# FJingxian/JanusX

Hardware: AMD Instinct MI355X
Metric: SNPs/sec full -lmm (GRM+eig+scan) (higher is better)
Workload: dtype f64 (eigendecomposition, REML and per-SNP statistics; GRM and rotation products are exact int8 / split-f16 MFMA sums merged in f64)

## Files before the change

janusx_amd/csrc/k_rotate_i8.hip:

```cpp
#include <stdlib.h>

#include "jx_common.h"

namespace jx {

typedef int i32x4 __attribute__((ext_vector_type(4)));
typedef int i32x16 __attribute__((ext_vector_type(16)));
typedef uint32_t u32x4q __attribute__((ext_vector_type(4)));

constexpr int RI_TM = 256;
constexpr int RI_TN = 128;
constexpr int RI_BK = 64;
constexpr int RI_IMG_A = RI_TM * RI_BK;
constexpr int RI_IMG_B = RI_TN * RI_BK;
constexpr int RI_SET = RI_IMG_A + 3 * RI_IMG_B;

__device__ __forceinline__ int ri_chunk_off(int row, int chunk) { return row * 64 + ((chunk ^ ((row >> 2) & 3)) << 4); }

__device__ __forceinline__ u32x4q ri_decode16(uint32_t w) {
    const uint32_t hi = (w >> 1) & 0x55555555u;
    const uint32_t v = hi + (hi & w);
    u32x4q o;
    o.x = v & 0x03030303u;
    o.y = (v >> 2) & 0x03030303u;
    o.z = (v >> 4) & 0x03030303u;
    o.w = (v >> 6) & 0x03030303u;
    return o;
}

__device__ __forceinline__ u32x4q ri_decode16_missing(uint32_t w) {
    const uint32_t v = w & ~(w >> 1) & 0x55555555u;
    u32x4q o;
    o.x = v & 0x03030303u;
    o.y = (v >> 2) & 0x03030303u;
    o.z = (v >> 4) & 0x03030303u;
    o.w = (v >> 6) & 0x03030303u;
    return o;
}

__global__ __launch_bounds__(256) void ut_rowmax_kernel(const float *__restrict__ ut, int n, int npad, float *__restrict__ umax) {
    const int j = blockIdx.x * 4 + (threadIdx.x >> 6), lane = threadIdx.x & 63;
    if (j >= npad) return;
    float a = 0.0f;
    if (j < n)
        for (int i = lane; i < n; i += 64) a = fmaxf(a, fabsf(ut[(int64_t)j * n + i]));
#pragma unroll
    for (int off = 32; off > 0; off >>= 1) a = fmaxf(a, __shfl_xor(a, off, 64));
    if (lane == 0) umax[j] = (a > 0.0f && a < 3.0e38f) ? a : 1.0f;
}

__global__ __launch_bounds__(256) void ut_quant3_kernel(const float *__restrict__ ut, int n, int64_t npad,
                                                        const float *__restrict__ umax, int8_t *__restrict__ q) {
    const int64_t idx = (int64_t)blockIdx.x * blockDim.x + threadIdx.x;
    const int64_t groups = npad / 16;
    if (idx >= npad * groups) return;
    const int64_t j = idx / groups, gq = idx - j * groups;
    int8_t o[3][16];
    const double inv = (j < n) ? 1.0 / (double)umax[j] : 0.0;
#pragma unroll
    for (int pos = 0; pos < 16; ++pos) {
        const int smp = ((pos & 3) << 2) | (pos >> 2);
        const int64_t i = gq * 16 + smp;
        double u = 0.0;
        if (j < n && i < n) u = (double)ut[j * (int64_t)n + i] * inv;
        const double a1 = u * 127.0;
        double q1 = rint(a1);
        const double a2 = (a1 - q1) * 254.0;
        double q2 = rint(a2);
        const double a3 = (a2 - q2) * 254.0;
        double q3 = rint(a3);
        q1 = fmin(fmax(q1, -127.0), 127.0);
        q2 = fmin(fmax(q2, -127.0), 127.0);
        q3 = fmin(fmax(q3, -127.0), 127.0);
        o[0][pos] = (int8_t)q1;
        o[1][pos] = (int8_t)q2;
        o[2][pos] = (int8_t)q3;
    }
#pragma unroll
    for (int pl = 0; pl < 3; ++pl)
        *reinterpret_cast<uint4 *>(q + pl * npad * npad + j * npad + gq * 16) = *reinterpret_cast<const uint4 *>(o[pl]);
}

template <int MODE>
__global__ __launch_bounds__(512, 2) void rotate_i8_kernel(const uint8_t *__restrict__ p32, int64_t m_total,
                                                           const int32_t *__restrict__ rows, int nrows,
                                                           const uint4 *__restrict__ lut16, const float *__restrict__ rowoff,
                                                           const float *__restrict__ usum, const int8_t *__restrict__ q,
                                                           const float *__restrict__ umax, int64_t npad, int n,
                                                           float *__restrict__ out, int64_t ldo,
                                                           const int32_t *__restrict__ sel) {
    extern __shared__ __attribute__((aligned(16))) uint8_t ri_smem[];
    float *sOff = reinterpret_cast<float *>(ri_smem + 2 * RI_SET);
    float *sSgn = sOff + RI_TM;
    int *sPos = reinterpret_cast<int *>(sSgn + RI_TM);

    const int tid = threadIdx.x, lane = tid & 63, wave = tid >> 6;
    const int wm = wave >> 2, wn = wave & 3;
    const int nrt = (nrows + RI_TM - 1) / RI_TM;
    const int xcd = blockIdx.x & 7, local = blockIdx.x >> 3;
    const int ct = (local / nrt) * 8 + xcd;
    if ((int64_t)ct * RI_TN >= npad) return;
    const int j0 = ct * RI_TN;
    const int r0 = (local % nrt) * RI_TM;

    const int arow = tid >> 1, ahalf = tid & 1;
    const uint8_t *arec = p32;
    int row_exact = 1;
    {
        const int r = r0 + arow;
        float boff = 0.0f, sgn = 1.0f;
        int pos = -1;
        if (r < nrows) {
            pos = sel ? sel[r] : r;
            const int64_t rec = rows ? (int64_t)rows[pos] : (int64_t)pos;
            arec = p32 + rec * 32;
            const float t = rowoff[pos];
            if (MODE == 1) {
                boff = t;
            } else {
                row_exact = (t == t) ? 1 : 0;
                const bool flipped = (lut16[pos].x & 0xffffu) != 0u;
                sgn = flipped ? -1.0f : 1.0f;
                boff = row_exact ? (t + (flipped ? 2.0f : 0.0f)) : 0.0f;
            }
        }
        if (ahalf == 0) {
            sOff[arow] = boff;
            sSgn[arow] = sgn;
            sPos[arow] = pos;
        }
    }
    if (__syncthreads_and(row_exact) == 0) return;
    arec += 8 * ahalf;

    const int brow = tid >> 2, bpart = tid & 3;
    const bool bok = j0 + brow < npad;
    const int8_t *bsrc = q + (int64_t)(bok ? j0 + brow : 0) * npad + bpart * 16;
    const uint32_t bmask = bok ? 0xffffffffu : 0u;
    const int64_t plane = npad * npad;
    const int boff_lds = ri_chunk_off(brow, bpart);

    uint2 wa = make_uint2(0, 0);
    u32x4q b0, b1, b2;
    auto load_a = [&](int kstep) {
        const int tile = kstep >> 1, sub = kstep & 1;
        wa = *reinterpret_cast<const uint2 *>(arec + (int64_t)tile * m_total * 32 + sub * 16);
    };
    auto load_b = [&](int64_t kcol) {
        b0 = *reinterpret_cast<const u32x4q *>(bsrc + kcol);
        b1 = *reinterpret_cast<const u32x4q *>(bsrc + plane + kcol);
        b2 = *reinterpret_cast<const u32x4q *>(bsrc + 2 * plane + kcol);
    };
    auto stage = [&](uint8_t *set) {
        *reinterpret_cast<u32x4q *>(set + ri_chunk_off(arow, 2 * ahalf)) = MODE == 1 ? ri_decode16_missing(wa.x) : ri_decode16(wa.x);
        *reinterpret_cast<u32x4q *>(set + ri_chunk_off(arow, 2 * ahalf + 1)) = MODE == 1 ? ri_decode16_missing(wa.y) : ri_decode16(wa.y);
        const u32x4q mk = {bmask, bmask, bmask, bmask};
        *reinterpret_cast<u32x4q *>(set + RI_IMG_A + boff_lds) = b0 & mk;
        *reinterpret_cast<u32x4q *>(set + RI_IMG_A + RI_IMG_B + boff_lds) = b1 & mk;
        *reinterpret_cast<u32x4q *>(set + RI_IMG_A + 2 * RI_IMG_B + boff_lds) = b2 & mk;
    };

    i32x16 acc[3][4];
#pragma unroll
    for (int pl = 0; pl < 3; ++pl)
#pragma unroll
        for (int mi = 0; mi < 4; ++mi)
#pragma unroll
            for (int r = 0; r < 16; ++r) acc[pl][mi][r] = 0;

    const int h = lane >> 5, frow = lane & 31;
    auto mfma_ks = [&](const uint8_t *set, int ks) {
        i32x4 b[3];
#pragma unroll
        for (int pl = 0; pl < 3; ++pl)
            b[pl] = *reinterpret_cast<const i32x4 *>(set + RI_IMG_A + pl * RI_IMG_B + ri_chunk_off(wn * 32 + frow, 2 * ks + h));
#pragma unroll
        for (int mp = 0; mp < 2; ++mp) {
            i32x4 a[2];
#pragma unroll
            for (int u = 0; u < 2; ++u)
                a[u] = *reinterpret_cast<const i32x4 *>(set + ri_chunk_off(wm * 128 + (2 * mp + u) * 32 + frow, 2 * ks + h));
#pragma unroll
            for (int u = 0; u < 2; ++u)
#pragma unroll
                for (int pl = 0; pl < 3; ++pl)
                    acc[pl][2 * mp + u] = __builtin_amdgcn_mfma_i32_32x32x32_i8(a[u], b[pl], acc[pl][2 * mp + u], 0, 0, 0);
            if (mp == 0) __builtin_amdgcn_sched_barrier(0);
        }
    };

    const int nk = (int)(npad / RI_BK);
    load_a(0);
    load_b(0);
    stage(ri_smem);
    {
        const int k1 = nk > 1 ? 1 : 0;
        load_a(k1);
        load_b((int64_t)k1 * RI_BK);
    }
    __syncthreads();
    int cur = 0;
    for (int ks = 0; ks < nk; ++ks) {
        const uint8_t *rd = ri_smem + cur * RI_SET;
        uint8_t *wr = ri_smem + (cur ^ 1) * RI_SET;
        const int kn = ks + 2 < nk ? ks + 2 : nk - 1;
        mfma_ks(rd, 0);
        stage(wr);
        load_a(kn);
        load_b((int64_t)kn * RI_BK);
        __builtin_amdgcn_sched_barrier(0);
        mfma_ks(rd, 1);
        __syncthreads();
        cur ^= 1;
    }

    const int gj = j0 + wn * 32 + frow;
    const bool colok = gj < n;
    const double um = colok ? (double)umax[gj] : 0.0;
    const double w1 = um / 127.0, w2 = um / (127.0 * 254.0), w3 = um / (127.0 * 254.0 * 254.0);
    const float us = (MODE == 0 && colok) ? usum[gj] : 0.0f;
#pragma unroll
    for (int mi = 0; mi < 4; ++mi) {
#pragma unroll
        for (int r = 0; r < 16; ++r) {
            const int lr = wm * 128 + mi * 32 + (r & 3) + 8 * (r >> 2) + 4 * h;
            const int gr = sPos[lr];
            if (gr >= 0 && colok) {
                const double v = (double)acc[0][mi][r] * w1 + (double)acc[1][mi][r] * w2 + (double)acc[2][mi][r] * w3;
                float *dst = out + (int64_t)gr * ldo + gj;
                if (MODE == 1) *dst = fmaf(sOff[lr], (float)v, *dst);
                else *dst = fmaf(sOff[lr], us, sSgn[lr] * (float)v);
            }
        }
    }
}

constexpr int RD_BK = 128;
constexpr int RD_A = 8 * 1024;
constexpr int RD_B = RI_TN * RD_BK;
constexpr int RD_STAGE = RD_A + 3 * RD_B;

__device__ __forceinline__ void rd_glds(const void *base, uint32_t off, unsigned lds_dst) {
    unsigned keep;
    const uint64_t b = (uint64_t)(uintptr_t)base;
    const uint32_t blo = __builtin_amdgcn_readfirstlane((uint32_t)b), bhi = __builtin_amdgcn_readfirstlane((uint32_t)(b >> 32));
    const uint64_t sb = ((uint64_t)bhi << 32) | blo;
    asm volatile("s_mov_b32 %0, m0\n\ts_mov_b32 m0, %3\n\ts_nop 0\n\tglobal_load_lds_dwordx4 %1, %2\n\ts_mov_b32 m0, %0"
                 : "=&s"(keep)
                 : "v"(off), "s"(sb), "s"(__builtin_amdgcn_readfirstlane(lds_dst))
                 : "memory");
}

template <int MODE> __device__ __forceinline__ i32x4 rd_decode(uint32_t w) {
    const u32x4q o = MODE == 1 ? ri_decode16_missing(w) : ri_decode16(w);
    i32x4 r;
    r.x = (int)o.x;
    r.y = (int)o.y;
    r.z = (int)o.z;
    r.w = (int)o.w;
    return r;
}

template <int MODE>
__global__ __launch_bounds__(512, 2) void rotate_i8_dma_kernel(const uint8_t *__restrict__ p32, int64_t m_total,
                                                               const int32_t *__restrict__ rows, int nrows,
                                                               const uint4 *__restrict__ lut16, const float *__restrict__ rowoff,
                                                               const float *__restrict__ usum, const int8_t *__restrict__ q,
                                                               const float *__restrict__ umax, int64_t npad, int n,
                                                               float *__restrict__ out, int64_t ldo,
                                                               const int32_t *__restrict__ sel) {
    extern __shared__ __attribute__((aligned(16))) uint8_t rd_smem[];
    float *sOff = reinterpret_cast<float *>(rd_smem + 2 * RD_STAGE);
    float *sSgn = sOff + RI_TM;
    int *sPos = reinterpret_cast<int *>(sSgn + RI_TM);

    const int tid = threadIdx.x, lane = tid & 63, wave = tid >> 6;
    const int wm = wave >> 2, wn = wave & 3;
    const int nrt = (nrows + RI_TM - 1) / RI_TM;
    const int xcd = blockIdx.x & 7, local = blockIdx.x >> 3;
    const int ct = (local / nrt) * 8 + xcd;
    if ((int64_t)ct * RI_TN >= npad) return;
    const int j0 = ct * RI_TN;
    const int r0 = (local % nrt) * RI_TM;

    uint32_t aoff = 0;
    int row_exact = 1;
    {
        const int arow = 32 * wave + (lane & 31);
        const int r = r0 + arow;
        float boff = 0.0f, sgn = 1.0f;
        int pos = -1;
        if (r < nrows) {
            pos = sel ? sel[r] : r;
            aoff = (uint32_t)(rows ? rows[pos] : pos) * 32u;
            const float t = rowoff[pos];
            if (MODE == 1) {
                boff = t;
            } else {
                row_exact = (t == t) ? 1 : 0;
                const bool flipped = (lut16[pos].x & 0xffffu) != 0u;
                sgn = flipped ? -1.0f : 1.0f;
                boff = row_exact ? (t + (flipped ? 2.0f : 0.0f)) : 0.0f;
            }
        }
        if (lane < 32) {
            sOff[arow] = boff;
            sSgn[arow] = sgn;
            sPos[arow] = pos;
        }
    }
    if (__syncthreads_and(row_exact) == 0) return;
    aoff += 16u * (uint32_t)(lane >> 5);

    uint32_t boffs[2];
#pragma unroll
    for (int e = 0; e < 2; ++e) {
        const int col = 16 * wave + 8 * e + (lane >> 3);
        const int c = (lane & 7) ^ ((col >> 1) & 7);
        boffs[e] = (uint32_t)col * (uint32_t)npad + (uint32_t)c * 16u;
    }
    const int8_t *qtile = q + (int64_t)j0 * npad;
    const int64_t plane = npad * npad;
    const int64_t atile = m_total * 32;
    const unsigned lds0 = (unsigned)(uintptr_t)rd_smem;
    auto issue = [&](int t, int buf) {
        const unsigned st = lds0 + buf * RD_STAGE;
        rd_glds(p32 + (int64_t)t * atile, aoff, st + wave * 1024);
#pragma unroll
        for (int pl = 0; pl < 3; ++pl)
#pragma unroll
            for (int e = 0; e < 2; ++e)
                rd_glds(qtile + pl * plane + (int64_t)t * RD_BK, boffs[e], st + RD_A + pl * RD_B + (2 * wave + e) * 1024);
    };

    i32x16 acc[3][4];
#pragma unroll
    for (int pl = 0; pl < 3; ++pl)
#pragma unroll
        for (int mi = 0; mi < 4; ++mi)
#pragma unroll
            for (int r = 0; r < 16; ++r) acc[pl][mi][r] = 0;

    const int h = lane >> 5, frow = lane & 31;
    const int afrag = wm * 4 * 1024 + h * 512 + frow * 16;
    const int bcol = (wn * 32 + frow) * RD_BK;
    const int bx0 = (4 * h) ^ ((frow >> 1) & 7);

    const int nk = (int)(npad / RD_BK);
    issue(0, 0);
    int buf = 0;
    for (int t = 0; t < nk; ++t) {
        asm volatile("s_waitcnt vmcnt(0)" ::: "memory");
        __builtin_amdgcn_s_barrier();
        asm volatile("" ::: "memory");
        issue(t + 1 < nk ? t + 1 : nk - 1, buf ^ 1);
        const uint8_t *st = rd_smem + buf * RD_STAGE;
        i32x4 araw[4];
#pragma unroll
        for (int mi = 0; mi < 4; ++mi) araw[mi] = *reinterpret_cast<const i32x4 *>(st + afrag + mi * 1024);
#pragma unroll
        for (int ks = 0; ks < 4; ++ks) {
            i32x4 b[3];
#pragma unroll
            for (int pl = 0; pl < 3; ++pl)
                b[pl] = *reinterpret_cast<const i32x4 *>(st + RD_A + pl * RD_B + bcol + ((bx0 ^ ks) << 4));
#pragma unroll
            for (int mi = 0; mi < 4; ++mi) {
                const i32x4 a = rd_decode<MODE>((uint32_t)araw[mi][ks]);
#pragma unroll
                for (int pl = 0; pl < 3; ++pl)
                    acc[pl][mi] = __builtin_amdgcn_mfma_i32_32x32x32_i8(a, b[pl], acc[pl][mi], 0, 0, 0);
            }
        }
        buf ^= 1;
    }
    asm volatile("s_waitcnt vmcnt(0)" ::: "memory");

    const int gj = j0 + wn * 32 + frow;
    const bool colok = gj < n;
    const double um = colok ? (double)umax[gj] : 0.0;
    const double w1 = um / 127.0, w2 = um / (127.0 * 254.0), w3 = um / (127.0 * 254.0 * 254.0);
    const float us = (MODE == 0 && colok) ? usum[gj] : 0.0f;
#pragma unroll
    for (int mi = 0; mi < 4; ++mi) {
#pragma unroll
        for (int r = 0; r < 16; ++r) {
            const int lr = wm * 128 + mi * 32 + (r & 3) + 8 * (r >> 2) + 4 * h;
            const int gr = sPos[lr];
            if (gr >= 0 && colok) {
                const double v = (double)acc[0][mi][r] * w1 + (double)acc[1][mi][r] * w2 + (double)acc[2][mi][r] * w3;
                float *dst = out + (int64_t)gr * ldo + gj;
                if (MODE == 1) *dst = fmaf(sOff[lr], (float)v, *dst);
                else *dst = fmaf(sOff[lr], us, sSgn[lr] * (float)v);
            }
        }
    }
}

static bool rot_i8_dma() {
    static const bool on = !(getenv("JXGPU_ROT_I8_DMA") && atoi(getenv("JXGPU_ROT_I8_DMA")) == 0);
    return on;
}

extern float g_last_ms[24];

}

using namespace jx;

namespace jx {
int launch_rotate_i8_missing(hipStream_t st, const uint8_t *d_p32, int64_t m_total, int n, const int32_t *d_rows, const int32_t *d_sel,
                             int nsel, const float *d_rowmiss, const int8_t *d_q, const float *d_umax, float *d_out, int64_t ld_out);
}
extern "C" int jxg_rotate_missing_dense(const uint8_t *d_p32, int64_t m_total, int n, const int32_t *d_rows, const int32_t *d_sel,
                                        int nsel, const float *d_rowmiss, const int8_t *d_q, const float *d_umax, float *d_out,
                                        int64_t ld_out, void *stream) {
    return launch_rotate_i8_missing((hipStream_t)stream, d_p32, m_total, n, d_rows, d_sel, nsel, d_rowmiss, d_q, d_umax, d_out, ld_out);
}

extern "C" int jxg_ut_quant3(const float *d_ut, int n, int8_t *d_q, float *d_umax, void *stream) {
    hipStream_t st = (hipStream_t)stream;
    const int64_t npad = (int64_t)num_tiles(n) * JXG_TILE;
    hipLaunchKernelGGL(ut_rowmax_kernel, dim3((unsigned)((npad + 3) / 4)), dim3(256), 0, st, d_ut, n, (int)npad, d_umax);
    JX_LAUNCH_CHECK();
    const int64_t items = npad * (npad / 16);
    if ((items + 255) / 256 > 0x7fffffffLL) return fail("jxg_ut_quant3: grid too large");
    hipLaunchKernelGGL(ut_quant3_kernel, dim3((unsigned)((items + 255) / 256)), dim3(256), 0, st, d_ut, n, npad, d_umax, d_q);
    JX_LAUNCH_CHECK();
    return 0;
}

namespace jx {
int launch_rotate_i8(hipStream_t st, const uint8_t *d_p32, int64_t m_total, int n, const int32_t *d_rows, const int32_t *d_sel,
                     int nsel, const void *d_lut16, const float *d_rowoff, const float *d_usum, const int8_t *d_q,
                     const float *d_umax, float *d_out, int64_t ld_out) {
    if (nsel <= 0) return 0;
    const int nt = num_tiles(n);
    const int64_t npad = (int64_t)nt * JXG_TILE;
    if (!d_q || !d_umax || !d_rowoff || !d_usum || n > 66000) return fail("launch_rotate_i8: planes missing or n > 66000");
    const int nrows = nsel;
    const int nct = (int)((npad + RI_TN - 1) / RI_TN), nrt = (nrows + RI_TM - 1) / RI_TM;
    static bool attr = false;
    const int lds = 2 * RI_SET + 3072;
    if (!attr) {
        JX_HIP(hipFuncSetAttribute((const void *)rotate_i8_kernel<0>, hipFuncAttributeMaxDynamicSharedMemorySize, lds));
        JX_HIP(hipFuncSetAttribute((const void *)rotate_i8_kernel<1>, hipFuncAttributeMaxDynamicSharedMemorySize, lds));
        attr = true;
    }
    dim3 grid((unsigned)(((nct + 7) / 8) * 8 * nrt));
    if (rot_i8_dma() && m_total < (1LL << 27)) {
        static bool attr_dma = false;
        const int lds_dma = 2 * RD_STAGE + 3072;
        if (!attr_dma) {
            JX_HIP(hipFuncSetAttribute((const void *)rotate_i8_dma_kernel<0>, hipFuncAttributeMaxDynamicSharedMemorySize, lds_dma));
            attr_dma = true;
        }
        hipLaunchKernelGGL(rotate_i8_dma_kernel<0>, grid, dim3(512), lds_dma, st, d_p32, m_total, d_rows, nrows,
                           (const uint4 *)d_lut16, d_rowoff, d_usum, d_q, d_umax, npad, n, d_out, ld_out, d_sel);
        JX_LAUNCH_CHECK();
        return 0;
    }
    hipLaunchKernelGGL(rotate_i8_kernel<0>, grid, dim3(512), lds, st, d_p32, m_total, d_rows, nrows, (const uint4 *)d_lut16,
                       d_rowoff, d_usum, d_q, d_umax, npad, n, d_out, ld_out, d_sel);
    JX_LAUNCH_CHECK();
    return 0;
}

int launch_rotate_i8_missing(hipStream_t st, const uint8_t *d_p32, int64_t m_total, int n, const int32_t *d_rows, const int32_t *d_sel,
                             int nsel, const float *d_rowmiss, const int8_t *d_q, const float *d_umax, float *d_out, int64_t ld_out) {
    if (nsel <= 0) return 0;
    const int nt = num_tiles(n);
    const int64_t npad = (int64_t)nt * JXG_TILE;
    if (!d_q || !d_umax || !d_rowmiss || !d_sel || n > 66000) return fail("launch_rotate_i8_missing: planes / list missing or n > 66000");
    const int nct = (int)((npad + RI_TN - 1) / RI_TN), nrt = (nsel + RI_TM - 1) / RI_TM;
    static bool attr = false;
    const int lds = 2 * RI_SET + 3072;
    if (!attr) {
        JX_HIP(hipFuncSetAttribute((const void *)rotate_i8_kernel<1>, hipFuncAttributeMaxDynamicSharedMemorySize, lds));
        attr = true;
    }
    dim3 grid((unsigned)(((nct + 7) / 8) * 8 * nrt));
    if (rot_i8_dma() && m_total < (1LL << 27)) {
        static bool attr_dma = false;
        const int lds_dma = 2 * RD_STAGE + 3072;
        if (!attr_dma) {
            JX_HIP(hipFuncSetAttribute((const void *)rotate_i8_dma_kernel<1>, hipFuncAttributeMaxDynamicSharedMemorySize, lds_dma));
            attr_dma = true;
        }
        hipLaunchKernelGGL(rotate_i8_dma_kernel<1>, grid, dim3(512), lds_dma, st, d_p32, m_total, d_rows, nsel,
                           (const uint4 *)nullptr, d_rowmiss, (const float *)nullptr, d_q, d_umax, npad, n, d_out, ld_out, d_sel);
        JX_LAUNCH_CHECK();
        return 0;
    }
    hipLaunchKernelGGL(rotate_i8_kernel<1>, grid, dim3(512), lds, st, d_p32, m_total, d_rows, nsel, (const uint4 *)nullptr,
                       d_rowmiss, (const float *)nullptr, d_q, d_umax, npad, n, d_out, ld_out, d_sel);
    JX_LAUNCH_CHECK();
    return 0;
}
}
```

janusx_amd/switches.py:

```python

SWITCHES = {
    "JXGPU_OZ_PLANES": ("numerics", "6 (5 inside pipeline.eigh_from_grm(f32_consumer=True))",
                        "digit planes of the sliced int8 products of the eigensolver (4..6); 4 is NOT a product state",
                        "test_sliced_int8_gemm[5|6], test_full_size_c2/c3/c4_properties[f32_consumer], test_end_to_end_two_stage"),
    "JXGPU_EIGH_F32_PLANES": ("numerics", "5", "0 keeps 6 planes for the f32-consuming pipeline",
                              "test_full_size_c3_properties[0.0-False] (6) / [0.0-True] (5)"),
    "JXGPU_STEDC_OZ_PLANES": ("numerics", "unset (follows JXGPU_OZ_PLANES)", "planes of the divide-and-conquer merges alone", "untested"),
    "JXGPU_GRM_MISS_DIGITS": ("numerics", "3", "2 = the two-digit dense missing-call GRM of rounds 4-5 (beta off by 1e-5..1e-4 end to end)",
                              "test_end_to_end_two_stage (default); 2 is NOT a product state"),
    "JXGPU_GRM_MISS": ("numerics", "1", "0: rows with missing calls on the fp16 split kernel (f32 accumulation, like the reference)",
                       "test_grm_missing_calls_sparse_correction"),
    "JXGPU_GRM_MISS_MAX": ("numerics", "0.012", "largest missing share for the sparse correction", "test_grm_missing_calls_sparse_correction"),
    "JXGPU_GRM_MISS_DENSE_MIN": ("numerics", "0.0015", "missing share from which the dense digit form replaces the sparse correction",
                                 "test_grm_missing_calls_sparse_correction, scripts/diag_e2e_two_stage.py"),
    "JXGPU_GRM_MISS_DENSE_ROWS": ("numerics", "16384", "fewest SNPs for the dense digit form", "test_grm_missing_calls_sparse_correction"),
    "JXGPU_GRM_FP4": ("form", "0", "1: the count Gram of the 256-tile form on the fp4 matrix pipes from a nibble image (exact like the int8 kernel)",
                      "test_grm_count_gram_on_the_fp4_pipes"),
    "JXGPU_GRM_I8": ("numerics", "1", "0: exact-integer SNPs on the fp16 single-product kernel (f32 sums instead of exact i32)", "untested"),
    "JXGPU_GRM_EXACT": ("numerics", "1", "0: every SNP on the fp16 hi/lo split kernel", "untested"),
    "JXGPU_ROT_I8": ("numerics", "1", "0: design rows on the fp16 hi/lo rotation instead of the exact int8 planes",
                     "test_full_size_rotation_kernels_with_mixed_rows"),
    "JXGPU_ROT_EXACT": ("numerics", "1", "0: no integer-LUT fast path in the fp16 rotation", "untested"),
    "JXGPU_ROT_MISS_DENSE": ("numerics", "auto", "form of the missing-call term of the int8 rotation (both exact)",
                             "test_rotation_rows_with_a_few_missing_calls_take_the_exact_path"),
    "JXGPU_ROT_MISS_MAX": ("numerics", "auto", "missing calls per row up to which the gather form is taken",
                           "test_rotation_rows_with_a_few_missing_calls_take_the_exact_path"),
    "JXGPU_PCG_I8": ("numerics", "1", "0: the PCG / HE operator halves on the f32 bit-plane table kernels (f32 partial sums per tile) instead of "
                     "exact int8 plane sums of a four-digit image of the vector", "test_pcg_operator_forms_agree"),
    "JXGPU_FVLMM_FUSED": ("numerics", "1", "0 / 2: unfused / always-fused fixed-lambda scan (f64 sums in a different order + f32 G~ round trip)",
                          "test_fixed_lambda_scan_fused_into_the_rotation_epilogue"),
    "JXGPU_SCAN_EXACT": ("numerics", "unset", "reference-formulation scan kernel instead of the tabulated one (1e-9 apart)",
                         "test_fast_scan_matches_exact_scan (through the entry points)"),
    "JXGPU_SCAN_SERIES": ("numerics", "1", "0: no per-SNP Chebyshev series (3e-16 apart)", "test_fast_scan_matches_exact_scan"),
    "JXGPU_SCAN_INTERP": ("numerics", "1", "0: Brent evaluates the tabulated objective directly instead of its per-SNP Chebyshev interpolant "
                          "(3.7e-15 apart; dim <= 4, series form only)",
                          "test_warm_start_chain_device_pipeline_matches_trajectories, test_fast_scan_matches_exact_scan, full-size legs"),
    "JXGPU_LMM2_EXACT": ("numerics", "unset", "LMM2 on the reference-formulation kernel", "test_lmm2_routes"),
    "JXGPU_EIGH": ("numerics", "auto", "onestage | twostage | rocsolver: which eigensolver (eigenvectors differ within 1e-10)",
                   "test_eigh_two_stage_path_and_its_fallback"),
    "JXGPU_EIGH_TWOSTAGE_MIN": ("numerics", "1500", "size from which the two-stage reduction runs", "test_eigh_two_stage_path_and_its_fallback"),
    "JXGPU_STEDC": ("numerics", "own", "rocsolver: vendor divide and conquer (diagnostic)", "test_eigh_own_divide_and_conquer"),
    "JXGPU_ORMTR": ("numerics", "own", "rocsolver back-transformation (diagnostic)", "untested"),
    "JXGPU_ORMTR_OZ": ("numerics", "1", "0: Q1 on the f64 MFMA GEMM instead of the sliced int8 one", "untested"),
    "JXGPU_STEDC_OZ": ("numerics", "1", "0: merges on the f64 MFMA GEMM", "untested"),
    "JXGPU_OZ_MIN_N": ("numerics", "3000 / 750", "size from which Q1 / the merges take the sliced products", "untested"),
    "JXGPU_DIST_BACKEND": ("knob", "nccl", "collective backend of `jx` multi-rank runs", "test_cli_two_ranks_share_one_gpu"),
    "JXGPU_DIST_EIGH": ("knob", "1", "0: replicated eigendecomposition on several ranks", "test_bench_two_ranks_share_one_gpu"),
    "JXGPU_DIST_EIGH_MIN_N": ("knob", "16384", "size from which the eigensolver's stages are dealt over the ranks", "test_bench_two_ranks_share_one_gpu"),
    "JXGPU_DIST_EIGH_ONESTAGE": ("knob", "unset", "sharded one-stage reduction", "untested"),
    "JXGPU_DIST_BAND": ("knob", "1", "0: band reduction replicated", "untested"),
    "JXGPU_DIST_BAND_MIN_N": ("knob", "16384", "size from which the band reduction is sharded", "test_sharded_band_reduction_rccl_single_rank"),
    "JXGPU_DIST_BAND_BLOCK": ("test", "auto", "block rows of the sharded band reduction", "test_sharded_band_reduction_rccl_single_rank"),
    "JXGPU_DIST_DC_WINDOW": ("knob", "1", "0: top-level merge replicated", "untested"),
    "JXGPU_SYR2K_PIPE_WGS": ("knob", "7/8 of the CUs", "workgroups of the persistent rank-2k update (the rest of the CUs serve the panel chain)",
                             "test_rank_2k_update_forms_give_the_same_bits"),
    "JXGPU_SPLMM_ROUTE": ("knob", "auto", "dense | block | factor: form of K + lambda I of the sparse-GRM routes",
                          "test_splmm_block_route_matches_the_dense_route, test_splmm_giant_component_both_sides_of_the_limit"),
    "JXGPU_SPLMM_BLOCK": ("knob", "4096", "samples per diagonal block of the block route", "test_splmm_block_route_matches_the_dense_route"),
    "JXGPU_SPLMM_BLOCK_MIN_N": ("knob", "16384", "size from which the block route is taken", "untested"),
    "JXGPU_SPGRM_ACC_GB": ("knob", "auto", "HBM for the sparse-GRM builder's accumulator", "untested"),
    "JXGPU_SPECTRAL_CACHE": ("knob", "1", "0: no reuse of the last sparse GRM's decomposition", "untested"),
    **{k: ("form", "default", "kernel / launch shape of the same computation", t) for k, t in {
        "JXGPU_BC_OWNED": "test_bulge_chasing_position_owned_equals_sweep_owned", "JXGPU_SB2ST_WGS": "untested", "JXGPU_GRM_I8_TILE": "test_sparse_grm_row_panels_write_the_same_file",
        "JXGPU_GRM_TILE": "untested", "JXGPU_GRM_EXACT_BK": "untested", "JXGPU_ROT256": "untested", "JXGPU_SCAN_NOLDS": "untested",
        "JXGPU_SCAN_NOTILE": "untested", "JXGPU_SBBACK_BAL": "untested", "JXGPU_SBBACK_BAL5": "test_eigh_balanced_q2_forms",
        "JXGPU_SBBACK_BAL_MIN": "untested", "JXGPU_SBBACK_BAL_PER": "untested", "JXGPU_SBBACK_GROUPS": "untested", "JXGPU_SBBACK_NW": "untested",
        "JXGPU_SBBACK_PAIR": "untested", "JXGPU_SBBACK_SOLO": "untested", "JXGPU_STEDC_LEAF": "test_eigh_own_divide_and_conquer",
        "JXGPU_STEDC_OWNLEAF": "untested", "JXGPU_STEDC_PAR": "untested", "JXGPU_STEDC_PARMIN": "untested", "JXGPU_SY2SB_LOOKAHEAD": "untested",
        "JXGPU_SYTRD_KT": "untested", "JXGPU_SYTRD_SYR2K": "untested", "JXGPU_SYTRD_TAIL": "untested", "JXGPU_SYTRD_TARGET": "untested",
        "JXGPU_DSYMM_SLOTS": "untested", "JXGPU_DSYMM_SPLIT": "untested", "JXGPU_ORMTR_NB": "untested",
        "JXGPU_ROT_I8_DMA": "test_int8_rotation_forms_give_the_same_bits",
        "JXGPU_SCAN_CHAIN_SPLIT": "test_warm_start_chain_kernels_on_rotated_rows_with_invalid_rows",
        "JXGPU_REPACK_WINDOW": "test_repack_of_a_sample_subset_window_form",
        "JXGPU_SYR2K_PIPE": "test_rank_2k_update_forms_give_the_same_bits",
        "JXGPU_KING_TILE": "test_fused_path_finds_every_finite_pair"}.items()},
    "JXGPU_QB_SKIP": ("test", "unset", "skips parts of the Q2 kernel (timing ablation; results are WRONG)", "test_q2_staggered_units_equal_lockstep (the lockstep value 64 only)"),
    "JXGPU_BC_SKIP": ("test", "unset", "bulge-chasing ablation (results WRONG)", "untested"),
    "JXGPU_BO_SLEEP": ("test", "unset", "hand-off delay of the bulge chasing (timing)", "untested"),
    "JXGPU_EIGH_TRACE": ("trace", "unset", "stage times of a decomposition to stderr", "-"),
    "JXGPU_PCG_TRACE": ("trace", "unset", "set-up marks of the PCG / HE / staging paths", "-"),
    "JXGPU_BENCH_BACKEND": ("test", "nccl", "bench.py: gloo for ranks sharing a GPU", "test_bench_two_ranks_share_one_gpu"),
    "JXGPU_BENCH_STEP_SLEEP_MS": ("test", "unset", "bench.py diagnostic: idle time in front of every odd step", "-"),
    "JXGPU_BENCH_CHILD": ("test", "unset", "bench.py: marks a child process", "-"),
    "JXGPU_BENCH_FORCE_DIST": ("test", "unset", "bench.py: one rank on the multi-rank code path", "test_distributed_eigh_rccl_callback_single_rank"),
    "JXGPU_DIST_EIGH_FORCE": ("test", "unset", "sharded eigensolver forms with one rank", "test_sharded_band_reduction_rccl_single_rank"),
    "JXGPU_DIST_EIGH_TEST_DISAGREE": ("test", "unset", "fault injection of the replica agreement check", "test_distributed_eigh_two_ranks_share_one_gpu"),
    "JXGPU_DIST_EIGH_TEST_DISAGREE2": ("test", "unset", "fault injection of the replica agreement check", "test_distributed_eigh_two_ranks_share_one_gpu"),
    "JXGPU_PCG_TEST_FAIL": ("test", "unset", "fault injection of the marker-sharded PCG", "test_marker_sharded_pcg_two_ranks_share_one_gpu"),
    "JXGPU_SCAN_CHAIN_FORCE_DIRECT": ("test", "unset", "row of a chain scan forced onto direct evaluations (its chain takes the one-kernel form)",
                                      "test_warm_start_chain_kernels_on_rotated_rows_with_invalid_rows"),
    "JXGPU_SPLMM_COMPONENT_MAX": ("test", "auto", "component limit of the spectral sparse routes", "test_splmm_giant_component_both_sides_of_the_limit"),
    "JXGPU_SPGRM_PANEL_ROWS": ("test", "auto", "row panels of the sparse-GRM builder", "test_sparse_grm_row_panels_write_the_same_file"),
}


def markdown_table(classes=("numerics",)):
    rows = ["| switch | product value | what another value does | covered by |", "|---|---|---|---|"]
    for name, (cls, default, what, test) in sorted(SWITCHES.items()):
        if cls in classes:
            cell = lambda t: str(t).replace(" | ", " / ").replace("|", "/")
            rows.append(f"| `{name}` | {cell(default)} | {cell(what)} | {cell(test)} |")
    return "\n".join(rows)
```

Baseline: 141,800.

## Add 512x64 rotation tile with grouped block order and interleaved DMA issue

The int8 rotation DMA kernel is templated on tile shape and gains a 512x64 tile, picked automatically when there are enough tiles to fill the device's CUs. Block-to-tile mapping for the narrow tile groups row and column tiles per XCD to improve L2 reuse. Next-stage global-to-LDS loads are now spread between the MFMA groups, with scheduling barriers, instead of issued all at once. The changed tile shape shifts the A/B reuse ratio and LDS size, which may affect occupancy, and blocks whose columns lie past n now exit early.

After: 143,200, median of 6. Within noise of the previous version (+1.0%).

```diff
diff --git a/janusx_amd/csrc/k_rotate_i8.hip b/janusx_amd/csrc/k_rotate_i8.hip
--- a/janusx_amd/csrc/k_rotate_i8.hip
+++ b/janusx_amd/csrc/k_rotate_i8.hip
@@ -1,4 +1,5 @@
 #include <stdlib.h>
+#include <string.h>
 
 #include "jx_common.h"
 
@@ -236,9 +237,17 @@
 }
 
 constexpr int RD_BK = 128;
-constexpr int RD_A = 8 * 1024;
-constexpr int RD_B = RI_TN * RD_BK;
-constexpr int RD_STAGE = RD_A + 3 * RD_B;
+
+template <int TM, int TN> struct RdTile {
+    static constexpr int WM = TM / 128, WN = TN / 32;
+    static constexpr int A = TM * 32;
+    static constexpr int B = TN * RD_BK;
+    static constexpr int STAGE = A + 3 * B;
+    static constexpr int NA = TM / 256;
+    static constexpr int NB = TN / 64;
+    static constexpr int LDS = 2 * STAGE + 3 * TM * 4;
+    static_assert(WM * WN == 8 && NA >= 1 && NB >= 1, "8 waves of 128 x 32");
+};
 
 __device__ __forceinline__ void rd_glds(const void *base, uint32_t off, unsigned lds_dst) {
     unsigned keep;
@@ -261,7 +270,7 @@
     return r;
 }
 
-template <int MODE>
+template <int MODE, int TM, int TN>
 __global__ __launch_bounds__(512, 2) void rotate_i8_dma_kernel(const uint8_t *__restrict__ p32, int64_t m_total,
                                                                const int32_t *__restrict__ rows, int nrows,
                                                                const uint4 *__restrict__ lut16, const float *__restrict__ rowoff,
@@ -269,38 +278,53 @@
                                                                const float *__restrict__ umax, int64_t npad, int n,
                                                                float *__restrict__ out, int64_t ldo,
                                                                const int32_t *__restrict__ sel) {
+    using T = RdTile<TM, TN>;
     extern __shared__ __attribute__((aligned(16))) uint8_t rd_smem[];
-    float *sOff = reinterpret_cast<float *>(rd_smem + 2 * RD_STAGE);
-    float *sSgn = sOff + RI_TM;
-    int *sPos = reinterpret_cast<int *>(sSgn + RI_TM);
+    float *sOff = reinterpret_cast<float *>(rd_smem + 2 * T::STAGE);
+    float *sSgn = sOff + TM;
+    int *sPos = reinterpret_cast<int *>(sSgn + TM);
 
     const int tid = threadIdx.x, lane = tid & 63, wave = tid >> 6;
-    const int wm = wave >> 2, wn = wave & 3;
-    const int nrt = (nrows + RI_TM - 1) / RI_TM;
+    const int wm = wave / T::WN, wn = wave % T::WN;
+    const int nrt = (nrows + TM - 1) / TM;
     const int xcd = blockIdx.x & 7, local = blockIdx.x >> 3;
-    const int ct = (local / nrt) * 8 + xcd;
-    if ((int64_t)ct * RI_TN >= npad) return;
-    const int j0 = ct * RI_TN;
-    const int r0 = (local % nrt) * RI_TM;
-
-    uint32_t aoff = 0;
+    int rt, ct;
+    if (TN == 64) {
+        const int srt = (nrt + 7) >> 3;
+        const int s = (local >> 5) * 8 + xcd, w = local & 31;
+        rt = (s % srt) * 8 + (w & 7);
+        ct = (s / srt) * 4 + (w >> 3);
+        if (rt >= nrt) return;
+    } else {
+        rt = local % nrt;
+        ct = (local / nrt) * 8 + xcd;
+    }
+    if ((int64_t)ct * TN >= npad) return;
+    const int j0 = ct * TN;
+    if (j0 >= n) return;
+    const int r0 = rt * TM;
+
+    uint32_t aoff[T::NA];
     int row_exact = 1;
-    {
-        const int arow = 32 * wave + (lane & 31);
+#pragma unroll
+    for (int e = 0; e < T::NA; ++e) {
+        const int arow = 32 * (wave + 8 * e) + (lane & 31);
         const int r = r0 + arow;
         float boff = 0.0f, sgn = 1.0f;
         int pos = -1;
+        aoff[e] = 0;
         if (r < nrows) {
             pos = sel ? sel[r] : r;
-            aoff = (uint32_t)(rows ? rows[pos] : pos) * 32u;
+            aoff[e] = (uint32_t)(rows ? rows[pos] : pos) * 32u;
             const float t = rowoff[pos];
             if (MODE == 1) {
                 boff = t;
             } else {
-                row_exact = (t == t) ? 1 : 0;
+                const int exact = (t == t) ? 1 : 0;
+                row_exact &= exact;
                 const bool flipped = (lut16[pos].x & 0xffffu) != 0u;
                 sgn = flipped ? -1.0f : 1.0f;
-                boff = row_exact ? (t + (flipped ? 2.0f : 0.0f)) : 0.0f;
+                boff = exact ? (t + (flipped ? 2.0f : 0.0f)) : 0.0f;
             }
         }
         if (lane < 32) {
@@ -308,14 +332,14 @@
             sSgn[arow] = sgn;
             sPos[arow] = pos;
         }
+        aoff[e] += 16u * (uint32_t)(lane >> 5);
     }
     if (__syncthreads_and(row_exact) == 0) return;
-    aoff += 16u * (uint32_t)(lane >> 5);
-
-    uint32_t boffs[2];
-#pragma unroll
-    for (int e = 0; e < 2; ++e) {
-        const int col = 16 * wave + 8 * e + (lane >> 3);
+
+    uint32_t boffs[T::NB];
+#pragma unroll
+    for (int e = 0; e < T::NB; ++e) {
+        const int col = 8 * (T::NB * wave + e) + (lane >> 3);
         const int c = (lane & 7) ^ ((col >> 1) & 7);
         boffs[e] = (uint32_t)col * (uint32_t)npad + (uint32_t)c * 16u;
     }
@@ -323,14 +347,15 @@
     const int64_t plane = npad * npad;
     const int64_t atile = m_total * 32;
     const unsigned lds0 = (unsigned)(uintptr_t)rd_smem;
-    auto issue = [&](int t, int buf) {
-        const unsigned st = lds0 + buf * RD_STAGE;
-        rd_glds(p32 + (int64_t)t * atile, aoff, st + wave * 1024);
-#pragma unroll
-        for (int pl = 0; pl < 3; ++pl)
-#pragma unroll
-            for (int e = 0; e < 2; ++e)
-                rd_glds(qtile + pl * plane + (int64_t)t * RD_BK, boffs[e], st + RD_A + pl * RD_B + (2 * wave + e) * 1024);
+    constexpr int NP = T::NA + 3 * T::NB;
+    auto issue_piece = [&](int t, int buf, int i) {
+        const unsigned st = lds0 + buf * T::STAGE;
+        if (i < T::NA) {
+            rd_glds(p32 + (int64_t)t * atile, aoff[i], st + (wave + 8 * i) * 1024);
+        } else {
+            const int pl = (i - T::NA) / T::NB, e = (i - T::NA) % T::NB;
+            rd_glds(qtile + pl * plane + (int64_t)t * RD_BK, boffs[e], st + T::A + pl * T::B + (T::NB * wave + e) * 1024);
+        }
     };
 
     i32x16 acc[3][4];
@@ -347,14 +372,15 @@
     const int bx0 = (4 * h) ^ ((frow >> 1) & 7);
 
     const int nk = (int)(npad / RD_BK);
-    issue(0, 0);
+#pragma unroll
+    for (int i = 0; i < NP; ++i) issue_piece(0, 0, i);
     int buf = 0;
     for (int t = 0; t < nk; ++t) {
         asm volatile("s_waitcnt vmcnt(0)" ::: "memory");
         __builtin_amdgcn_s_barrier();
         asm volatile("" ::: "memory");
-        issue(t + 1 < nk ? t + 1 : nk - 1, buf ^ 1);
-        const uint8_t *st = rd_smem + buf * RD_STAGE;
+        const int tn = t + 1 < nk ? t + 1 : nk - 1;
+        const uint8_t *st = rd_smem + buf * T::STAGE;
         i32x4 araw[4];
 #pragma unroll
         for (int mi = 0; mi < 4; ++mi) araw[mi] = *reinterpret_cast<const i32x4 *>(st + afrag + mi * 1024);
@@ -363,13 +389,18 @@
             i32x4 b[3];
 #pragma unroll
             for (int pl = 0; pl < 3; ++pl)
-                b[pl] = *reinterpret_cast<const i32x4 *>(st + RD_A + pl * RD_B + bcol + ((bx0 ^ ks) << 4));
+                b[pl] = *reinterpret_cast<const i32x4 *>(st + T::A + pl * T::B + bcol + ((bx0 ^ ks) << 4));
 #pragma unroll
             for (int mi = 0; mi < 4; ++mi) {
                 const i32x4 a = rd_decode<MODE>((uint32_t)araw[mi][ks]);
 #pragma unroll
                 for (int pl = 0; pl < 3; ++pl)
                     acc[pl][mi] = __builtin_amdgcn_mfma_i32_32x32x32_i8(a, b[pl], acc[pl][mi], 0, 0, 0);
+                if (ks * 4 + mi < NP) {
+                    __builtin_amdgcn_sched_barrier(0);
+                    issue_piece(tn, buf ^ 1, ks * 4 + mi);
+                    __builtin_amdgcn_sched_barrier(0);
+                }
             }
         }
         buf ^= 1;
@@ -400,6 +431,63 @@
 static bool rot_i8_dma() {
     static const bool on = !(getenv("JXGPU_ROT_I8_DMA") && atoi(getenv("JXGPU_ROT_I8_DMA")) == 0);
     return on;
+}
+
+constexpr int RD_WIDE_MIN_ROUNDS = 1;
+
+static int rot_i8_tile_switch() {
+    const char *e = getenv("JXGPU_ROT_I8_TILE");
+    if (!e || !*e) return 0;
+    if (!strcmp(e, "256x128")) return 1;
+    if (!strcmp(e, "512x64")) return 2;
+    return -1;
+}
+
+static int device_cus() {
+    static int cus = 0;
+    if (!cus) {
+        int dev = 0;
+        hipDeviceProp_t prop;
+        if (hipGetDevice(&dev) != hipSuccess || hipGetDeviceProperties(&prop, dev) != hipSuccess) return 256;
+        cus = prop.multiProcessorCount > 0 ? prop.multiProcessorCount : 256;
+    }
+    return cus;
+}
+
+static bool rot_i8_tile_512(int nrows, int n) {
+    return (int64_t)((nrows + 511) / 512) * ((n + 63) / 64) >= (int64_t)RD_WIDE_MIN_ROUNDS * device_cus();
+}
+
+template <int MODE, int TM, int TN>
+static int launch_rd(hipStream_t st, const uint8_t *d_p32, int64_t m_total, const int32_t *d_rows, int nrows, const uint4 *d_lut16,
+                     const float *d_rowoff, const float *d_usum, const int8_t *d_q, const float *d_umax, int64_t npad, int n,
+                     float *d_out, int64_t ld_out, const int32_t *d_sel) {
+    using T = RdTile<TM, TN>;
+    static bool attr = false;
+    if (!attr) {
+        JX_HIP(hipFuncSetAttribute((const void *)rotate_i8_dma_kernel<MODE, TM, TN>, hipFuncAttributeMaxDynamicSharedMemorySize, T::LDS));
+        attr = true;
+    }
+    const int64_t nct = (npad + TN - 1) / TN, nrt = (nrows + TM - 1) / TM;
+    const int64_t wgs = TN == 64 ? ((((nrt + 7) / 8) * ((nct + 3) / 4) + 7) / 8) * 8 * 32 : ((nct + 7) / 8) * 8 * nrt;
+    if (wgs > 0x7fffffffLL) return fail("rotate_i8: grid too large");
+    hipLaunchKernelGGL((rotate_i8_dma_kernel<MODE, TM, TN>), dim3((unsigned)wgs), dim3(512), T::LDS, st, d_p32, m_total, d_rows, nrows,
+                       d_lut16, d_rowoff, d_usum, d_q, d_umax, npad, n, d_out, ld_out, d_sel);
+    JX_LAUNCH_CHECK();
+    return 0;
+}
+
+template <int MODE>
+static int launch_rd_tile(hipStream_t st, const uint8_t *d_p32, int64_t m_total, const int32_t *d_rows, int nrows, const uint4 *d_lut16,
+                          const float *d_rowoff, const float *d_usum, const int8_t *d_q, const float *d_umax, int64_t npad, int n,
+                          float *d_out, int64_t ld_out, const int32_t *d_sel) {
+    const int sw = rot_i8_tile_switch();
+    if (sw < 0) return fail("JXGPU_ROT_I8_TILE: 256x128 or 512x64");
+    if (sw ? sw == 2 : rot_i8_tile_512(nrows, n))
+        return launch_rd<MODE, 512, 64>(st, d_p32, m_total, d_rows, nrows, d_lut16, d_rowoff, d_usum, d_q, d_umax, npad, n, d_out, ld_out,
+                                        d_sel);
+    return launch_rd<MODE, 256, 128>(st, d_p32, m_total, d_rows, nrows, d_lut16, d_rowoff, d_usum, d_q, d_umax, npad, n, d_out, ld_out,
+                                     d_sel);
 }
 
 extern float g_last_ms[24];
@@ -448,18 +536,9 @@
         attr = true;
     }
     dim3 grid((unsigned)(((nct + 7) / 8) * 8 * nrt));
-    if (rot_i8_dma() && m_total < (1LL << 27)) {
-        static bool attr_dma = false;
-        const int lds_dma = 2 * RD_STAGE + 3072;
-        if (!attr_dma) {
-            JX_HIP(hipFuncSetAttribute((const void *)rotate_i8_dma_kernel<0>, hipFuncAttributeMaxDynamicSharedMemorySize, lds_dma));
-            attr_dma = true;
-        }
-        hipLaunchKernelGGL(rotate_i8_dma_kernel<0>, grid, dim3(512), lds_dma, st, d_p32, m_total, d_rows, nrows,
-                           (const uint4 *)d_lut16, d_rowoff, d_usum, d_q, d_umax, npad, n, d_out, ld_out, d_sel);
-        JX_LAUNCH_CHECK();
-        return 0;
-    }
+    if (rot_i8_dma() && m_total < (1LL << 27))
+        return launch_rd_tile<0>(st, d_p32, m_total, d_rows, nrows, (const uint4 *)d_lut16, d_rowoff, d_usum, d_q, d_umax, npad, n, d_out,
+                                 ld_out, d_sel);
     hipLaunchKernelGGL(rotate_i8_kernel<0>, grid, dim3(512), lds, st, d_p32, m_total, d_rows, nrows, (const uint4 *)d_lut16,
                        d_rowoff, d_usum, d_q, d_umax, npad, n, d_out, ld_out, d_sel);
     JX_LAUNCH_CHECK();
@@ -480,18 +559,9 @@
         attr = true;
     }
     dim3 grid((unsigned)(((nct + 7) / 8) * 8 * nrt));
-    if (rot_i8_dma() && m_total < (1LL << 27)) {
-        static bool attr_dma = false;
-        const int lds_dma = 2 * RD_STAGE + 3072;
-        if (!attr_dma) {
-            JX_HIP(hipFuncSetAttribute((const void *)rotate_i8_dma_kernel<1>, hipFuncAttributeMaxDynamicSharedMemorySize, lds_dma));
-            attr_dma = true;
-        }
-        hipLaunchKernelGGL(rotate_i8_dma_kernel<1>, grid, dim3(512), lds_dma, st, d_p32, m_total, d_rows, nsel,
-                           (const uint4 *)nullptr, d_rowmiss, (const float *)nullptr, d_q, d_umax, npad, n, d_out, ld_out, d_sel);
-        JX_LAUNCH_CHECK();
-        return 0;
-    }
+    if (rot_i8_dma() && m_total < (1LL << 27))
+        return launch_rd_tile<1>(st, d_p32, m_total, d_rows, nsel, (const uint4 *)nullptr, d_rowmiss, (const float *)nullptr, d_q, d_umax,
+                                 npad, n, d_out, ld_out, d_sel);
     hipLaunchKernelGGL(rotate_i8_kernel<1>, grid, dim3(512), lds, st, d_p32, m_total, d_rows, nsel, (const uint4 *)nullptr,
                        d_rowmiss, (const float *)nullptr, d_q, d_umax, npad, n, d_out, ld_out, d_sel);
     JX_LAUNCH_CHECK();
diff --git a/janusx_amd/switches.py b/janusx_amd/switches.py
--- a/janusx_amd/switches.py
+++ b/janusx_amd/switches.py
@@ -70,6 +70,7 @@
         "JXGPU_SYTRD_KT": "untested", "JXGPU_SYTRD_SYR2K": "untested", "JXGPU_SYTRD_TAIL": "untested", "JXGPU_SYTRD_TARGET": "untested",
         "JXGPU_DSYMM_SLOTS": "untested", "JXGPU_DSYMM_SPLIT": "untested", "JXGPU_ORMTR_NB": "untested",
         "JXGPU_ROT_I8_DMA": "test_int8_rotation_forms_give_the_same_bits",
+        "JXGPU_ROT_I8_TILE": "test_rotation_tiles_give_the_same_bits, test_rotation_tile_rows_do_not_depend_on_their_neighbours",
         "JXGPU_SCAN_CHAIN_SPLIT": "test_warm_start_chain_kernels_on_rotated_rows_with_invalid_rows",
         "JXGPU_REPACK_WINDOW": "test_repack_of_a_sample_subset_window_form",
         "JXGPU_SYR2K_PIPE": "test_rank_2k_update_forms_give_the_same_bits",
```
